# bleyerj/dolfinx_materials

Hardware: AMD Instinct MI355X
Metric: M quadrature-point updates/s (stress+tangent, fp64) (higher is better)
Workload: dtype f64; 1 GPU; cfg2: J2 von-Mises plasticity, linear isotropic hardening, small strain, 1e+07 Gauss points per GPU, stress + 6x6 consistent tangent, load/unload history increments 2-4; points_per_gpu=10000000, law=j2_linear, layout=AoS (N,6)/(N,36) boundary arrays in HBM, SoA resident state, placement=every array where its first allocation put it, settle_launches_before_warmup=540

## Files before the change

dolfinx_materials_amd/_lib.py:

```python
from __future__ import annotations

import ctypes as C
import os
import subprocess

_HERE = os.path.dirname(os.path.abspath(__file__))
LIB_PATH = os.environ.get("DXM_LIB_PATH") or os.path.join(_HERE, "libdxmat.so")
CSRC_DIR = os.path.join(_HERE, "csrc")

DXM_MAX_STATE_FIELDS = 4
LAW_ELASTIC_ISO, LAW_J2_LINEAR, LAW_J2_VOCE, LAW_FEFP_J2_VOCE, LAW_FEFP_J2_LINEAR = 0, 1, 2, 3, 4
LAW_RAMBERG_OSGOOD = 5
LAW_OGDEN = 7
LAW_HOSFORD_LINEAR = 10
LAW_ORTHOTROPIC_ELASTIC = 12
S0, S1 = 0, 1


class DxmError(RuntimeError):
    """Hard error reported by libdxmat (negative return code)."""


class LawInfo(C.Structure):
    _fields_ = [
# ... 41 lines not shown
    "dxm_destroy": (C.c_int, [_h]),
    "dxm_npoints": (C.c_int64, [_h]),
    "dxm_law": (C.c_int, [_h]),
    "dxm_set_params": (C.c_int, [_h, _dp, C.c_int]),
    "dxm_set_param_field": (C.c_int, [_h, C.c_int, C.c_void_p]),
    "dxm_set_param_field_device": (C.c_int, [_h, C.c_int, C.c_void_p, C.c_void_p]),
    "dxm_param_field_mask": (C.c_int, [_h]),
    "dxm_set_frame": (C.c_int, [_h, C.c_void_p]),
    "dxm_set_frame_field": (C.c_int, [_h, C.c_void_p]),
    "dxm_set_frame_field_device": (C.c_int, [_h, C.c_void_p, C.c_void_p]),
    "dxm_frame_kind": (C.c_int, [_h]),
    "dxm_algorithmic_bytes": (C.c_int, [_h]),
    "dxm_set_newton": (C.c_int, [_h, C.c_int, C.c_double]),
    "dxm_set_tangent_layout": (C.c_int, [_h, C.c_int]),
    "dxm_tangent_size": (C.c_int, [_h]),
    "dxm_set_state": (C.c_int, [_h, C.c_int, C.c_int, C.c_void_p]),
    "dxm_get_state": (C.c_int, [_h, C.c_int, C.c_int, C.c_void_p]),
    "dxm_advance": (C.c_int, [_h]),
    "dxm_revert": (C.c_int, [_h]),
    "dxm_io_held": (C.c_int, [_h, C.c_int]),
    "dxm_get_io": (C.c_int, [_h, C.c_int, C.c_int, C.c_void_p]),
    "dxm_integrate_rows": (C.c_int, [_h, C.c_void_p, C.c_double, C.c_void_p, C.c_void_p, C.c_void_p, C.POINTER(Stats)]),
    "dxm_integrate": (
        C.c_int,
        [_h, C.c_void_p, C.c_double, C.c_void_p, C.c_void_p, C.c_void_p, C.POINTER(Stats)],
    ),
    "dxm_integrate_device": (
        C.c_int,
        [_h, C.c_void_p, C.c_double, C.c_void_p, C.c_void_p, C.c_void_p],
    ),
    "dxm_get_stats": (C.c_int, [_h, C.POINTER(Stats)]),
    "dxm_isv_device": (C.c_int, [_h, C.c_int, C.c_void_p, C.c_void_p]),
    "dxm_state_ptr": (C.c_void_p, [_h, C.c_int, C.c_int, C.c_int]),
    "dxm_integrate_displacement_device": (C.c_int, [_h, _h, C.c_void_p, C.c_double, C.c_void_p, C.c_void_p, C.c_void_p]),
    "dxm_expand_tangent_device": (C.c_int, [C.c_void_p, C.c_int64, C.c_void_p, C.c_int, C.c_void_p]),
    "dxm_expand_tangent_pack4_device": (C.c_int, [C.c_void_p, C.c_void_p, C.c_int64, C.c_void_p, C.c_int, C.c_void_p]),
    "dxm_kernel_name": (C.c_char_p, [_h]),
    "dxm_launch_generation": (C.c_uint64, [_h]),
    "dxm_notify_replay": (C.c_int, [_h]),
    "dxm_set_option": (C.c_int, [_h, C.c_char_p, C.c_double]),
    "dxm_isv_host": (C.c_int, [_h, C.c_int, C.c_void_p]),
    "dxm_bind_isv_output": (C.c_int, [_h, C.c_int, C.c_void_p]),
    "dxm_host_copy": (C.c_int, [C.c_void_p, C.c_void_p, C.c_uint64, C.c_int]),
    "dxm_host_scatter_rows": (C.c_int, [C.c_void_p, C.c_void_p, C.c_void_p, C.c_int64, C.c_int, C.c_int]),
    "dxm_host_gather_rows": (C.c_int, [C.c_void_p, C.c_void_p, C.c_void_p, C.c_int64, C.c_int, C.c_int]),
    "dxm_host_index_range": (C.c_int, [C.c_void_p, C.c_int64, C.c_int, C.POINTER(C.c_int64), C.POINTER(C.c_int64)]),
    "dxm_host_register": (C.c_int, [C.c_void_p, C.c_uint64]),
    "dxm_host_unregister": (C.c_int, [C.c_void_p]),
    "dxm_host_alloc": (C.c_void_p, [C.c_uint64]),
    "dxm_host_free": (C.c_int, [C.c_void_p]),
    "dxm_mesh_create_hex8": (_h, [C.c_void_p, C.c_int64, C.c_void_p, C.c_int64, C.c_void_p, C.c_int, C.c_int]),
    "dxm_mesh_create_tet4": (_h, [C.c_void_p, C.c_int64, C.c_void_p, C.c_int64, C.c_int, C.c_int]),
    "dxm_mesh_create_simplex": (
        _h,
        [C.c_int, C.c_void_p, C.c_int64, C.c_void_p, C.c_int64, C.c_void_p, C.c_int, C.c_int64, C.c_void_p, C.c_int, C.c_int],
    ),
    "dxm_mesh_destroy": (C.c_int, [_h]),
    "dxm_mesh_npoints": (C.c_int64, [_h]),
    "dxm_mesh_displacement_size": (C.c_int64, [_h]),
    "dxm_mesh_gradient_device": (C.c_int, [_h, C.c_void_p, C.c_int, C.c_void_p, C.c_void_p]),
    "dxm_integrate_displacement": (
        C.c_int,
        [_h, _h, C.c_void_p, C.c_double, C.c_void_p, C.c_void_p, C.c_void_p, C.POINTER(Stats)],
    ),
    "dxm_integrate_displacement_rows": (
        C.c_int,
# ... 197 lines not shown
```

dolfinx_materials_amd/csrc/dxmat.hip:

```cpp
#include <hip/hip_runtime.h>

#include <algorithm>
#include <atomic>
#include <chrono>
#include <cmath>
#include <condition_variable>
#include <deque>
#include <map>
#include <mutex>
#include <thread>
#include <cstdarg>
#include <cstdio>
#include <cstdlib>
#include <cstring>
#include <string>
#include <vector>

#include "../../include/dxmat.h"
#include "dxm_common.hpp"
#include "fefp.hpp"
#include "gradient.hpp"
#include "small_strain.hpp"
#include "ramberg_osgood.hpp"
#include "param_fields.hpp"
#include "hyperelastic.hpp"
#include "hosford.hpp"
#include "orthotropic.hpp"
#include "host_side.hpp"

using namespace dxm;
static_assert(TL_FULL == DXM_TANGENT_FULL && TL_SYM == DXM_TANGENT_SYM && TL_COEF == DXM_TANGENT_COEF && TL_PACK4 == DXM_TANGENT_PACK4, "kernel and ABI layout ids");

static thread_local std::string g_last_error;

static int fail(int code, const char* fmt, ...) {
  char buf[512];
  va_list ap;
  va_start(ap, fmt);
  vsnprintf(buf, sizeof(buf), fmt, ap);
  va_end(ap);
  g_last_error = buf;
  return code;
}

#define HIP_TRY(expr)                                                                      \
  do {                                                                                     \
    hipError_t _e = (expr);                                                                \
    if (_e != hipSuccess) {                                                                \
      (void)hipGetLastError();                                                             \
      return fail(-2, "%s failed: %s (%s:%d)", #expr, hipGetErrorString(_e), __FILE__, __LINE__); \
    }                                                                                      \
  } while (0)

struct DeviceGuard {
  int prev = -1;
  bool ok = true;
// ... 444 lines not shown
  double* h_coef = nullptr;
  int h_coef_per_point = 0;
  double* h_flux = nullptr;
  double* h_isv = nullptr;
  double elastic_lm[2] = {0.0, 0.0};
  hipEvent_t chunk_done[DXM_MAX_CHUNKS] = {};
  hipEvent_t kernel_done[DXM_MAX_CHUNKS] = {};
  int num_cu = 256;
  int blocks_per_cu = 5;
  int tangent_layout = 0;
  double* d_grad = nullptr;
  double* d_flux = nullptr;
  double* d_grad0 = nullptr;
  double* d_flux0 = nullptr;
  int io1_valid = 0;
  int io0_valid = 0;
  int opt_keep_initial_io = 0;
  double* d_isv = nullptr;
  double* isv_out[DXM_MAX_STATE_FIELDS] = {};
  double* d_isv_fields = nullptr;
  double* d_ct = nullptr;
  double* d_field = nullptr;
  double* h_grad_ring = nullptr;
  int64_t ring_slot_doubles = 0;
  hipEvent_t ring_done[DXM_RING] = {};
  int opt_stage_ahead = 3;
  double unregister_ms = 0.0;
  int pf_mask = 0;
  double* pf_law[2] = {nullptr, nullptr};
  double* pf_stream[PF_COUNT] = {};
  int frame_kind = 0;
  Frame9 frame_uniform{};
  double* frame_streams = nullptr;
};

static int sync_last(dxm_material* m);
static int pf_refresh_elastic(dxm_material* m, hipStream_t st);

static void free_state(dxm_material* m) {
  if (!m->state_base) return;
  (void)hipFree(m->state_base);
  m->state_base = nullptr;
}

static int build_params(dxm_material* m, const double* p, int np) {
  const LawDesc& d = kLaws[m->law];
  const int expect = n_params_of(d);
  if (np != expect) return fail(-1, "law %d expects %d parameters, got %d", m->law, expect, np);
  LawParams q{};
  q.maxit = m->maxit;
  q.rtol = m->rtol;
  if (int rc = d.build(p, q)) return rc;
  m->prm = q;
  m->raw_params.assign(p, p + np);
  return 0;
}

static int tangent_size(const dxm_material* m) {
  const LawDesc& d = kLaws[m->law];
  if (m->tangent_layout == DXM_TANGENT_SYM) return d.n_flux * (d.n_flux + 1) / 2;
  if (m->tangent_layout == DXM_TANGENT_COEF) return 9;
  if (m->tangent_layout == DXM_TANGENT_PACK4) return 4;
  return d.n_flux * d.n_grad;
}

__global__ void fill_slot_kernel(double* dst, int64_t count, double value) {
  const int64_t i = (int64_t)blockIdx.x * blockDim.x + threadIdx.x;
  if (i < count) dst[i] = value;
}

struct PackMap { int n; int slot[16]; };

// ... 100 lines not shown
  if (hipStreamCreateWithFlags(&m->own_stream, hipStreamNonBlocking) != hipSuccess ||
      hipEventCreateWithFlags(&m->last_event, hipEventDisableTiming) != hipSuccess) {
    fail(-2, "hipStreamCreate / hipEventCreate failed"); return bail();
  }
  if (d.n_slots > 0) {
    const size_t bytes = (size_t)d.n_slots * m->ld * sizeof(double);
    {
      if (hipMalloc(&m->state_base, 2 * bytes + m->s1_skew) != hipSuccess) {
        fail(-3, "hipMalloc of %zu state bytes failed", 2 * bytes + m->s1_skew); return bail();
      }
      m->state[0] = m->state_base;
      m->state[1] = reinterpret_cast<double*>(reinterpret_cast<char*>(m->state_base) + bytes + m->s1_skew);
    }
  }
  {
    hipFuncAttributes fa;
    if (d.residency_kernel && hipFuncGetAttributes(&fa, d.residency_kernel()) == hipSuccess && fa.numRegs > 0) {
      const int alloc = ((fa.numRegs + 7) / 8) * 8;
      int waves_simd = 512 / alloc;
      if (waves_simd > 8) waves_simd = 8;
      int by_vgpr = waves_simd * 4 / WAVES_PER_BLOCK;
      int by_lds = fa.sharedSizeBytes > 0 ? (int)(160 * 1024 / fa.sharedSizeBytes) : 8;
      int occ = by_vgpr < by_lds ? by_vgpr : by_lds;
      if (occ < 1) occ = 1;
      m->blocks_per_cu = occ;
    }
    if (d.blocks_per_cu) m->blocks_per_cu = d.blocks_per_cu;
  }
  m->stats_capacity = dxm_host::stats_capacity(m->num_cu, npoints);
  if (hipMalloc(&m->d_stats, sizeof(BlockStats) * m->stats_capacity) != hipSuccess) {
    fail(-3, "hipMalloc of stats failed"); return bail();
  }
  if (init_state(m) != 0) return bail();
  g_last_error.clear();
  return m;
}

int dxm_destroy(dxm_material* m) {
  if (!m) return 0;
  DeviceGuard guard(m->device);
  (void)sync_last(m);
  delete m->pool;
  if (m->h_coef) (void)hipHostFree(m->h_coef);
  if (m->h_flux) (void)hipHostFree(m->h_flux);
  if (m->h_isv) (void)hipHostFree(m->h_isv);
  for (hipEvent_t e : m->chunk_done) if (e) (void)hipEventDestroy(e);
  for (hipEvent_t e : m->kernel_done) if (e) (void)hipEventDestroy(e);
  if (m->last_event) (void)hipEventDestroy(m->last_event);
  free_state(m);
  if (m->d_stats) (void)hipFree(m->d_stats);
  if (m->h_stats) (void)hipHostFree(m->h_stats);
  if (m->d_grad) (void)hipFree(m->d_grad);
  if (m->d_flux) (void)hipFree(m->d_flux);
  if (m->d_grad0) (void)hipFree(m->d_grad0);
  if (m->d_flux0) (void)hipFree(m->d_flux0);
  if (m->d_isv) (void)hipFree(m->d_isv);
  if (m->d_isv_fields) (void)hipFree(m->d_isv_fields);
  if (m->d_ct) (void)hipFree(m->d_ct);
  if (m->d_field) (void)hipFree(m->d_field);
  if (m->h_grad_ring) (void)hipHostFree(m->h_grad_ring);
  for (double* q : m->pf_law) if (q) (void)hipFree(q);
  for (double* q : m->pf_stream) if (q) (void)hipFree(q);
  if (m->frame_streams) (void)hipFree(m->frame_streams);
  for (hipEvent_t e : m->ring_done) if (e) (void)hipEventDestroy(e);
  if (m->own_stream) (void)hipStreamDestroy(m->own_stream);
  if (m->pipe_stream) (void)hipStreamDestroy(m->pipe_stream);
// ... 36 lines not shown
  if (maxit < 1 || !(rtol > 0.0)) return fail(-1, "invalid Newton controls maxit=%d rtol=%g", maxit, rtol);
  m->maxit = maxit;
  m->rtol = rtol;
  if (int rc = build_params(m, m->raw_params.data(), (int)m->raw_params.size())) return rc;
  ++m->epoch;
  return 0;
}

static int check_field(const dxm_material* m, int which, int field) {
  if (!m) return fail(-1, "null handle");
  if (which != DXM_S0 && which != DXM_S1) return fail(-1, "state selector must be DXM_S0 or DXM_S1");
  const LawDesc& d = kLaws[m->law];
  if (field < 0 || field >= d.n_fields) return fail(-1, "law %d has no state field %d", m->law, field);
  return 0;
}

static int sync_last(dxm_material* m) {
  if (!m->launched) return 0;
  if (m->last_event_recorded) {
    HIP_TRY(hipEventSynchronize(m->last_event));
  } else {
    HIP_TRY(hipDeviceSynchronize());
  }
  return 0;
}

static double* state_of(const dxm_material* m, int which) {
  return m->state[(which == DXM_S1 && !m->s1_alias) ? 1 : 0];
}

static int materialize_s1(dxm_material* m) {
  if (!m->s1_alias) return 0;
  const LawDesc& d = kLaws[m->law];
  if (d.n_slots > 0)
    HIP_TRY(hipMemcpy(m->state[1], m->state[0], (size_t)d.n_slots * m->ld * sizeof(double),
                      hipMemcpyDeviceToDevice));
  m->s1_alias = false;
  return 0;
}


constexpr size_t BOUNCE_BYTES = 16u << 20;
static dxm_host::LockedTable g_locked;
static std::atomic<int> g_query_foreign{1};
static void note_locked(const void* p, size_t bytes) { g_locked.note(p, bytes); }
static void forget_locked(const void* p) { g_locked.forget(p); }
static bool in_locked_table(const void* host, size_t bytes) { return g_locked.contains(host, bytes); }
static bool page_locked_byte(const void* host) {
  hipPointerAttribute_t attr{};
  const bool locked = host && hipPointerGetAttributes(&attr, host) == hipSuccess && attr.type == hipMemoryTypeHost;
  (void)hipGetLastError();
  return locked;
}
static bool page_locked(const void* host, size_t bytes) {
  if (!host) return false;
  if (in_locked_table(host, bytes)) return true;
  if (!g_query_foreign.load()) return false;
  if (!page_locked_byte(host)) return false;
  return bytes <= 1 || page_locked_byte(static_cast<const char*>(host) + bytes - 1);
}
struct Staging {
  char* buf = nullptr;
  hipEvent_t done[2] = {nullptr, nullptr};
};
static std::mutex g_staging_mu[64];
static Staging g_staging[64];
// ... 53 lines not shown
  if (int rc = current_device_index(&devi)) return rc;
  std::lock_guard<std::mutex> lk(g_staging_mu[devi]);
  Staging* s = nullptr;
  if (int rc = staging_for_current_device(&s)) return rc;
  const size_t nchunks = (bytes + BOUNCE_BYTES - 1) / BOUNCE_BYTES;
  for (size_t c = 0; c < nchunks; ++c) {
    if (c >= 2) HIP_TRY(hipEventSynchronize(s->done[c & 1]));
    memcpy(s->buf + (c & 1) * BOUNCE_BYTES, static_cast<const char*>(host) + c * BOUNCE_BYTES, chunk_size(c, nchunks, bytes));
    HIP_TRY(hipMemcpyAsync(static_cast<char*>(dev) + c * BOUNCE_BYTES, s->buf + (c & 1) * BOUNCE_BYTES, chunk_size(c, nchunks, bytes),
                           hipMemcpyHostToDevice, st));
    HIP_TRY(hipEventRecord(s->done[c & 1], st));
  }
  HIP_TRY(hipStreamSynchronize(st));
  return 0;
}

int dxm_set_state(dxm_material* m, int which, int field, const double* host_aos) {
  if (int rc = check_field(m, which, field)) return rc;
  if (!host_aos) return fail(-1, "null host pointer");
  DEVICE_GUARD(m);
  if (int rc = sync_last(m)) return rc;
  const LawDesc& d = kLaws[m->law];
  const int dim = d.isv_dim[field];
  const int64_t n = m->n;
  if (n == 0) return 0;
  if (int rc = materialize_s1(m)) return rc;
  if (!m->d_field) HIP_TRY(hipMalloc(&m->d_field, sizeof(double) * n * 6));
  PackMap map{};
  map.n = dim;
  for (int c = 0; c < dim; ++c) map.slot[c] = d.isv_slot[field] + c;
  hipStream_t st = m->own_stream;
  if (int rc = upload_from_host(m->d_field, host_aos, sizeof(double) * n * dim, st)) return rc;
  const int blocks = (int)((n * dim + 255) / 256);
  hipLaunchKernelGGL(unpack_isv_kernel, dim3(blocks), dim3(256), 0, st, state_of(m, which), m->ld, n,
                     m->d_field, map);
  HIP_TRY(hipGetLastError());
  HIP_TRY(hipStreamSynchronize(st));
  return 0;
}

int dxm_get_state(dxm_material* m, int which, int field, double* host_aos) {
  if (int rc = check_field(m, which, field)) return rc;
  if (!host_aos) return fail(-1, "null host pointer");
  DEVICE_GUARD(m);
  if (int rc = sync_last(m)) return rc;
  const LawDesc& d = kLaws[m->law];
  const int dim = d.isv_dim[field];
  const int64_t n = m->n;
  if (n == 0) return 0;
  if (!m->d_field) HIP_TRY(hipMalloc(&m->d_field, sizeof(double) * n * 6));
  PackMap map{};
  map.n = dim;
  for (int c = 0; c < dim; ++c) map.slot[c] = d.isv_slot[field] + c;
  hipStream_t st = m->own_stream;
  const int blocks = (int)((n * dim + 255) / 256);
  hipLaunchKernelGGL(pack_isv_kernel, dim3(blocks), dim3(256), 0, st, state_of(m, which), m->ld, n,
                     m->d_field, map);
  HIP_TRY(hipGetLastError());
  return download_to_host(host_aos, m->d_field, sizeof(double) * n * dim, st);
}

int dxm_advance(dxm_material* m) {
  if (!m) return fail(-1, "null handle");
  if (!m->s1_alias) {
    double* t = m->state[0];
    m->state[0] = m->state[1];
// ... 27 lines not shown
  if (!host_aos) return fail(-1, "null host pointer");
  DEVICE_GUARD(m);
  if (int rc = sync_last(m)) return rc;
  const LawDesc& d = kLaws[m->law];
  const bool first = which == DXM_S0 || m->s1_alias;
  const double* src = kind ? (first ? m->d_flux0 : m->d_flux) : (first ? m->d_grad0 : m->d_grad);
  return download_to_host(host_aos, src, sizeof(double) * m->n * (kind ? d.n_flux : d.n_grad), m->own_stream);
}

int dxm_revert(dxm_material* m) {
  if (!m) return fail(-1, "null handle");
  m->s1_alias = true;
  m->io1_valid = 0;
  return 0;
}

}

template <int LAW>
static void launch_small_strain(const LaunchArgs& a) {
  dxm_material* m = a.m;
  const int grid = a.grid, tl = a.tl;
  const hipStream_t st = a.st;
  const int64_t cnt = a.cnt;
  const double* grad = a.grad;
  double *flux = a.flux, *ct = a.ct;
  const double* s0 = m->state[0] + a.off;
  double* s1 = m->state[1] + a.off;
  BlockStats* bs = m->d_stats + a.stats_off;
  const MeshSource none{};
  const MeshSource& src = a.fused ? *a.fused : none;
  const int g = a.fused ? a.fused->kind : 0;
  constexpr int dyn_lds = LAW == LAW_ELASTIC ? 0 : 2304;
#ifndef DXM_CUSTOM_HARDENING
  if constexpr (LAW != LAW_ELASTIC) {
    if (m->pf_mask) {
      ParamStreams pf{};
      for (int k = 0; k < PF_COUNT; ++k) pf.p[k] = m->pf_stream[k] ? m->pf_stream[k] + a.off : nullptr;
      param_fields_launch(LAW, tl, g, grid, dyn_lds, st, m->prm, pf, cnt, grad, s0, s1, m->ld, flux, ct, bs, src);
      return;
    }
  }
#endif
#define DXM_LAUNCH_SS(TL, G)                                                                              \
  hipLaunchKernelGGL((small_strain_kernel<LAW, TL, G>), dim3(grid), dim3(BLOCK), dyn_lds, st, m->prm, cnt, grad, s0, s1, \
                     m->ld, flux, ct, bs, src)
#define DXM_LAUNCH_SS_G(TL) do { if (g == 0) DXM_LAUNCH_SS(TL, 0); else if (g == 1) DXM_LAUNCH_SS(TL, 1); \
                                 else if (g == 2) DXM_LAUNCH_SS(TL, 2); else DXM_LAUNCH_SS(TL, 3); } while (0)
  if (tl == TL_SYM) DXM_LAUNCH_SS_G(TL_SYM);
  else if (tl == TL_FULL) DXM_LAUNCH_SS_G(TL_FULL);
  else if constexpr (ss_has_coef<LAW>) { if (tl == TL_PACK4) DXM_LAUNCH_SS_G(TL_PACK4); else DXM_LAUNCH_SS_G(TL_COEF); }
#undef DXM_LAUNCH_SS_G
#undef DXM_LAUNCH_SS
}

static void launch_fefp(const LaunchArgs& a, bool voce) {
  dxm_material* m = a.m;
  const int grid = a.grid;
  const hipStream_t st = a.st;
  const int64_t cnt = a.cnt;
  const double* grad = a.grad;
  double *flux = a.flux, *ct = a.ct;
  const double* s0 = m->state[0] + a.off;
  double* s1 = m->state[1] + a.off;
  BlockStats* bs = m->d_stats + a.stats_off;
  const MeshSource none{};
// ... 737 lines not shown

int dxm_integrate_displacement_rows(dxm_material* m, dxm_mesh* mesh, const double* u_host, double dt, double* flux_rows,
                                    double* ct_rows, const int64_t* rows, dxm_stats* stats) {
  (void)dt;
  if (!m) return fail(-1, "null argument");
  if (m->n > 0 && (!flux_rows || !ct_rows || !rows)) return fail(-1, "dxm_integrate_displacement_rows needs the flux array, the tangent array and the row index");
  return integrate_displacement_host(m, mesh, u_host, flux_rows, nullptr, ct_rows, stats, rows);
}

int dxm_integrate_displacement_device(dxm_material* m, dxm_mesh* mesh, const double* u_dev, double dt,
                                      double* flux_dev, double* ct_dev, void* hip_stream) {
  (void)dt;
  if (!m || !mesh) return fail(-1, "null argument");
  if (mesh->device != m->device) return fail(-1, "mesh and material live on different devices");
  if (dxm_mesh_npoints(mesh) != m->n) return fail(-1, "mesh has %lld Gauss points, material %lld",
                                                   (long long)dxm_mesh_npoints(mesh), (long long)m->n);
  if (m->n > 0 && (!u_dev || !flux_dev || !ct_dev)) return fail(-1, "null device pointer");
  DEVICE_GUARD(m);
  hipStream_t st = (hipStream_t)hip_stream;
  const LawDesc& d = kLaws[m->law];
  if (m->opt_fused_gradient && fusable(mesh)) {
    const MeshSource src = mesh_source(mesh, u_dev);
    return launch(m, flux_dev , flux_dev, ct_dev, st, &src);
  }
  if (!m->d_grad) HIP_TRY(hipMalloc(&m->d_grad, sizeof(double) * m->n * d.n_grad));
  if (int rc = dxm_mesh_gradient_device(mesh, u_dev, gradient_kind(d), m->d_grad, hip_stream)) return rc;
  return launch(m, m->d_grad, flux_dev, ct_dev, st);
}

const double* dxm_state_ptr(const dxm_material* m, int which, int field, int comp) {
  if (check_field(m, which, field)) return nullptr;
  const LawDesc& d = kLaws[m->law];
  if (comp < 0 || comp >= d.isv_dim[field]) { fail(-1, "component out of range"); return nullptr; }
  return state_of(m, which) + (size_t)(d.isv_slot[field] + comp) * m->ld;
}

const char* dxm_kernel_name(const dxm_material* m) {
  if (!m) return "";
  if (m->frame_kind) return kLaws[m->law].frame_kernel[m->frame_kind - 1];
  return m->pf_mask ? kLaws[m->law].field_kernel : kLaws[m->law].kernel;
}

int dxm_expand_tangent_device(const double* coef_dev, int64_t npoints, double* ct_dev, int device, void* hip_stream) {
  if (npoints < 0) return fail(-1, "negative point count");
  if (npoints == 0) return 0;
  if (!coef_dev || !ct_dev) return fail(-1, "null device pointer");
  if (((uintptr_t)coef_dev | (uintptr_t)ct_dev) & 15) return fail(-1, "coefficient / tangent device arrays must be 16-byte aligned");
  DeviceGuard guard(device);
  if (!guard.ok) return fail(-2, "hipSetDevice(%d) failed", device);
  const int64_t tiles = (npoints + WAVE - 1) / WAVE;
  int64_t blocks = (tiles + WAVES_PER_BLOCK - 1) / WAVES_PER_BLOCK;
  if (blocks > 256 * 32) blocks = 256 * 32;
  hipLaunchKernelGGL(expand_tangent_kernel, dim3((unsigned)blocks), dim3(BLOCK), 0, (hipStream_t)hip_stream, npoints, coef_dev, ct_dev);
  HIP_TRY(hipGetLastError());
  return 0;
}

int dxm_expand_tangent_pack4_device(const double* flux_dev, const double* pack_dev, int64_t npoints, double* ct_dev, int device,
                                    void* hip_stream) {
  if (npoints < 0) return fail(-1, "negative point count");
  if (npoints == 0) return 0;
  if (!flux_dev || !pack_dev || !ct_dev) return fail(-1, "null device pointer");
  if (((uintptr_t)flux_dev | (uintptr_t)pack_dev | (uintptr_t)ct_dev) & 15) return fail(-1, "stress / pack / tangent device arrays must be 16-byte aligned");
  DeviceGuard guard(device);
  if (!guard.ok) return fail(-2, "hipSetDevice(%d) failed", device);
  const int64_t tiles = (npoints + WAVE - 1) / WAVE;
  int64_t blocks = (tiles + WAVES_PER_BLOCK - 1) / WAVES_PER_BLOCK;
// ... 204 lines not shown

int dxm_set_frame_field_device(dxm_material* m, const double* dev_aos, void* hip_stream) {
  if (int rc = frame_check(m)) return rc;
  if (!dev_aos) return dxm_set_frame_field(m, nullptr);
  DEVICE_GUARD(m);
  hipStream_t st = (hipStream_t)hip_stream;
  if (m->launched && m->last_event_recorded) HIP_TRY(hipStreamWaitEvent(st, m->last_event, 0));
  else if (int rc = sync_last(m)) return rc;
#ifndef DXM_CUSTOM_HARDENING
  if (int rc = frame_reserve(m)) return rc;
  orthotropic_frames_to_streams(m->n, dev_aos, m->frame_streams, m->ld, st);
  HIP_TRY(hipGetLastError());
#endif
  m->frame_kind = 2;
  ++m->epoch;
  return 0;
}

int dxm_frame_kind(const dxm_material* m) { return m ? m->frame_kind : -1; }

int dxm_algorithmic_bytes(const dxm_material* m) {
  if (!m) return -1;
  int bytes = kLaws[m->law].alg_bytes;
  for (const double* q : m->pf_stream) if (q) bytes += 8;
  if (m->frame_kind == 2) bytes += 9 * 8;
  return bytes;
}

int dxm_notify_replay(dxm_material* m) {
  if (!m) return fail(-1, "null handle");
  m->launched = true;
  m->last_event_recorded = false;
  m->s1_alias = false;
  return 0;
}

uint64_t dxm_launch_generation(const dxm_material* m) { return m ? (m->epoch << 1) | (uint64_t)m->parity : 0; }

int dxm_set_option(dxm_material* m, const char* name, double value) {
  if (!m || !name) return fail(-1, "null argument");
  const std::string k(name);
  const bool on = value != 0.0;
  if (k == "pipeline") m->opt_pipeline = on;
  else if (k == "split_streams") m->opt_split_streams = on;
  else if (k == "packed_transfer") {
    if (!(value == 0.0 || value == 1.0 || value == 2.0)) return fail(-1, "packed_transfer must be 0, 1 or 2");
    m->opt_packed_transfer = (int)value;
  }
  else if (k == "fused_gradient") m->opt_fused_gradient = on;
  else if (k == "verbose") m->opt_verbose = on;
  else if (k == "stage_ahead") {
    if (!(value >= 1 && value <= DXM_RING - 2)) return fail(-1, "stage_ahead must be in [1, %d]", DXM_RING - 2);
    m->opt_stage_ahead = (int)value;
  }
  else if (k == "register_input") {
    if (!(value == 0.0 || value == 1.0 || value == 2.0)) return fail(-1, "register_input must be 0, 1 or 2");
    m->up.set_option((int)value);
  }
  else if (k == "keep_initial_io") m->opt_keep_initial_io = on;
  else if (k == "pageable_dma") m->opt_pageable_dma = value != 0.0;
  else if (k == "query_foreign_pointers") g_query_foreign.store(on ? 1 : 0);
  else if (k == "packed_min_points") {
    if (!(value >= 0 && value <= 1e12)) return fail(-1, "packed_min_points must be >= 0");
    m->opt_packed_min_points = (int64_t)value;
  }
  else if (k == "host_threads") {
    if (!(value >= 1 && value <= 256)) return fail(-1, "host_threads must be in [1, 256]");
    m->opt_host_threads = (int)value;
  } else if (k == "max_chunks") {
    if (!(value >= 1 && value <= DXM_MAX_CHUNKS)) return fail(-1, "max_chunks must be in [1, %d]", DXM_MAX_CHUNKS);
    m->opt_max_chunks = (int)value;
  } else if (k == "blocks_per_cu") {
    if (!(value >= 1 && value <= 256)) return fail(-1, "blocks_per_cu must be in [1, 256]");
    m->blocks_per_cu = (int)value;
  } else {
    return fail(-1, "unknown option '%s'", name);
  }
  ++m->epoch;
  return 0;
}

int dxm_isv_host(dxm_material* m, int which, double* isv_aos) {
  if (!m) return fail(-1, "null handle");
  if (which != DXM_S0 && which != DXM_S1) return fail(-1, "state selector must be DXM_S0 or DXM_S1");
  const LawDesc& d = kLaws[m->law];
  const int total = isv_total(d);
  if (total == 0 || m->n == 0) return 0;
  if (!isv_aos) return fail(-1, "null host pointer");
  DEVICE_GUARD(m);
  if (int rc = sync_last(m)) return rc;
  if (!m->d_isv) HIP_TRY(hipMalloc(&m->d_isv, sizeof(double) * m->n * total));
  if (int rc = pack_isv_range(m, which, 0, m->n, m->d_isv, m->own_stream)) return rc;
  return download_to_host(isv_aos, m->d_isv, sizeof(double) * m->n * total, m->own_stream);
}

int dxm_host_copy(void* dst, const void* src, uint64_t bytes, int threads) {
  if (bytes == 0) return 0;
  if (!dst || !src) return fail(-1, "null host pointer");
  dxm_host::host_copy(dst, src, bytes, threads);
  return 0;
}

static int move_rows(bool scatter, double* dst, const double* src, const int64_t* rows, int64_t n, int width, int threads) {
  if (n <= 0 || width <= 0) return 0;
  if (!dst || !src || !rows) return fail(-1, "null host pointer");
  dxm_host::move_rows(scatter, dst, src, rows, n, width, threads);
  return 0;
// ... 38 lines not shown
```

dolfinx_materials_amd/csrc/host_side.hpp:

```cpp
#pragma once

#include <algorithm>
#include <atomic>
#include <cmath>
#include <condition_variable>
#include <cstdint>
#include <cstring>
#include <deque>
#include <map>
#include <mutex>
#include <thread>
#include <vector>

#include "../../include/dxmat.h"

namespace dxm_host {

typedef double double2_h __attribute__((ext_vector_type(2)));

constexpr double THIRD = 1.0 / 3.0;
constexpr int MAX_CHUNKS = 64;
constexpr int RING = 16;
constexpr int FEFP_RECORD = 54;

// ... 229 lines not shown
};

struct ChunkPlan {
  int nchunks;
  int64_t csize;
  int64_t offset(int c) const { return (int64_t)c * csize; }
  int64_t count(int c, int64_t n) const {
    const int64_t o = offset(c);
    return o >= n ? 0 : ((n - o) < csize ? (n - o) : csize);
  }
  int issued(int64_t n) const { return csize > 0 ? (int)std::min<int64_t>(nchunks, (n + csize - 1) / csize) : 0; }
};

inline ChunkPlan plan_chunks(int64_t n, bool packed, bool staged_upload, int max_chunks, bool pipeline) {
  int nchunks = (int)std::min<int64_t>(n / (packed ? (n >= 2097152 ? 65536 : 32768) : 131072), MAX_CHUNKS * 1024);
  if (nchunks < 1) nchunks = 1;
  if (!packed && nchunks > (staged_upload ? 32 : 8)) nchunks = staged_upload ? 32 : 8;
  if (nchunks > max_chunks) nchunks = max_chunks;
  if (nchunks > MAX_CHUNKS) nchunks = MAX_CHUNKS;
  if (!pipeline) nchunks = 1;
  const int64_t csize = ((n + nchunks - 1) / nchunks + 255) / 256 * 256;
  return ChunkPlan{nchunks, csize};
}

inline int ring_slot(int chunk) { return chunk % RING; }

inline int stats_capacity(int num_cu, int64_t npoints) {
  return (int)std::min<int64_t>(INT32_MAX, std::max<int64_t>((int64_t)num_cu * 256, (npoints + 255) / 256 + MAX_CHUNKS));
}
inline int launch_grid(int64_t cnt, int num_cu, int blocks_per_cu) {
  const int64_t tiles = (cnt + 255) / 256;
  const int64_t cap = (int64_t)num_cu * blocks_per_cu;
  return (int)std::max<int64_t>(1, std::min<int64_t>(tiles, cap));
}

struct TransferRequest {
  int law;
  int n_grad, n_flux, n_isv_fields, isv_dim[DXM_MAX_STATE_FIELDS];
  int layout, tangent_size;
  int64_t n;
  bool flux, isv_aos, ct;
  bool rows;
  bool staged_grad;
  bool fused;
  unsigned bound_fields;
  bool flux_locked, isv_locked, ct_locked;
  int packed_transfer;
  int64_t packed_min_points;
  bool split_streams, pipeline;
  int max_chunks;
};

enum class Route { none, dma, staged, rows };
enum class CtRoute { none, fill, dma, staged, rebuild, rows_move, rows_rebuild, rows_fill };

struct TransferPlan {
  TransferRequest req;
  bool packed;
  int tl;
  int nt;
  int np;
  int land;
  int nfull;
  int job;
  CtRoute ct;
  Route flux, isv, fields;
// ... 227 lines not shown
```

dolfinx_materials_amd/csrc/small_strain.hpp:

```cpp
#pragma once
#include "dxm_common.hpp"
#include "gradient.hpp"
#include "param_fields.hpp"

namespace dxm {

enum { LAW_ELASTIC = 0, LAW_J2_LINEAR = 1, LAW_J2_VOCE = 2, LAW_RAMBERG_OSGOOD = 3 };

template <int LAW> constexpr bool ss_has_state = LAW == LAW_J2_LINEAR || LAW == LAW_J2_VOCE;
template <int LAW> constexpr bool ss_has_coef = LAW != LAW_ELASTIC;

constexpr int RO_I3MU = 0, RO_BETA = 1, RO_ISIG0 = 2, RO_N = 3, RO_INVN = 4, RO_ESIG = 5;
constexpr double RO_EPS = 1e-12;

constexpr int SS_NSLOTS = 7;

constexpr int SS_STAGE = 64 * 6;
constexpr int SS_COEF = 64 * 9;
constexpr int SS_LDS_PER_WAVE = SS_STAGE + SS_COEF;
static_assert(8 * HEX_FUSED_REC <= SS_COEF, "the 8 cell records of a fused tile live in the coefficient region");

template <int LAW>
__device__ __forceinline__ double hardening_R(const LawParams& prm, double p) {
  if constexpr (LAW == LAW_J2_LINEAR) {
// ... 77 lines not shown
  const double d[6] = {et[0] - third, et[1] - third, et[2] - third, et[3], et[4], et[5]};
  const double g = se * (2.0 / 3.0) / fmax(eq, RO_EPS);
  const double ktr = prm.kappa * tr;
  s[0] = ktr + g * d[0];
  s[1] = ktr + g * d[1];
  s[2] = ktr + g * d[2];
  s[3] = g * d[3];
  s[4] = g * d[4];
  s[5] = g * d[5];
}

__device__ __forceinline__ double2_t tangent_pair(const double* cf, int i, int j) {
  const double k1 = cf[0], k2 = cf[1], k3 = cf[2];
  const double ni = cf[3 + i], nj0 = cf[3 + j], nj1 = cf[4 + j];
  const double t0 = ((i < 3 && j < 3) ? k1 : 0.0) + ((i == j) ? k2 : 0.0);
  const double t1 = ((i < 3 && j + 1 < 3) ? k1 : 0.0) + ((i == j + 1) ? k2 : 0.0);
  double2_t v;
  v.x = t0 + k3 * (ni * nj0);
  v.y = t1 + k3 * (ni * nj1);
  return v;
}

enum { TL_FULL = 0, TL_SYM = 1, TL_COEF = 2, TL_PACK4 = 3 };
constexpr double SS_THIRD = 1.0 / 3.0;

template <int LAW, int TL, int GRAD = 0>
__global__ void __launch_bounds__(BLOCK, 4)
small_strain_kernel(const LawParams prm, const int64_t n, const double* __restrict__ eps,
                    const double* __restrict__ s0, double* __restrict__ s1, const int64_t ld,
                    double* __restrict__ sig, double* __restrict__ ct,
                    BlockStats* __restrict__ stats, const MeshSource src) {
  constexpr bool FIELDS = false;
  constexpr ParamStreams pf = {};
#include "small_strain_body.hpp"
}

template <int LAW, int TL, int GRAD = 0>
__global__ void __launch_bounds__(BLOCK, 4)
small_strain_field_kernel(const LawParams prm, const ParamStreams pf, const int64_t n, const double* __restrict__ eps,
                          const double* __restrict__ s0, double* __restrict__ s1, const int64_t ld,
                          double* __restrict__ sig, double* __restrict__ ct,
                          BlockStats* __restrict__ stats, const MeshSource src) {
  static_assert(LAW == LAW_J2_LINEAR || LAW == LAW_J2_VOCE, "parameter fields: the J2 laws");
  constexpr bool FIELDS = true;
#include "small_strain_body.hpp"
}

#ifndef DXM_UPDATE_KERNELS_ONLY
__global__ void __launch_bounds__(BLOCK, 4)
expand_tangent_kernel(const int64_t n, const double* __restrict__ cin, double* __restrict__ ct) {
  __shared__ __attribute__((aligned(16))) double lds_all[WAVES_PER_BLOCK * SS_COEF];
  const int lane = threadIdx.x & (WAVE - 1);
  const int wid = threadIdx.x >> 6;
  double* coef = lds_all + wid * SS_COEF;
  const int64_t ntiles = (n + WAVE - 1) / WAVE;
  for (int64_t tile = (int64_t)blockIdx.x * WAVES_PER_BLOCK + wid; tile < ntiles; tile += (int64_t)gridDim.x * WAVES_PER_BLOCK) {
    const int64_t base = tile * WAVE;
    const int npts = (n - base) < WAVE ? (int)(n - base) : WAVE;
    if (npts == WAVE) {
      const double2_t* g = reinterpret_cast<const double2_t*>(cin + base * 9);
      double2_t v[5];
#pragma unroll
      for (int k = 0; k < 5; ++k) v[k] = (k * WAVE + lane < 288) ? g[k * WAVE + lane] : double2_t{0.0, 0.0};
#pragma unroll
      for (int k = 0; k < 5; ++k)
        if (k * WAVE + lane < 288) reinterpret_cast<double2_t*>(coef)[k * WAVE + lane] = v[k];
    } else {
#pragma unroll
      for (int k = 0; k < 9; ++k) {
        const int idx = k * WAVE + lane;
        coef[idx] = idx < npts * 9 ? cin[base * 9 + idx] : 0.0;
      }
    }
    wave_lds_sync();
#include "small_strain_expand_store.hpp"
    wave_lds_sync();
  }
// ... 46 lines not shown
```

dolfinx_materials_amd/csrc/small_strain_body.hpp:

```cpp
  __shared__ __attribute__((aligned(16))) double lds_all[WAVES_PER_BLOCK * SS_LDS_PER_WAVE];
  __shared__ unsigned long long red[4 * WAVES_PER_BLOCK];

  int lane = threadIdx.x & (WAVE - 1);
  const int wid = threadIdx.x >> 6;
  double* stage = lds_all + wid * SS_LDS_PER_WAVE;
  double* coef = stage + SS_STAGE;
  double2_t* stage2 = reinterpret_cast<double2_t*>(stage);

  const int64_t ntiles = (n + WAVE - 1) / WAVE;
  const int64_t tile_stride = (int64_t)gridDim.x * WAVES_PER_BLOCK;

  unsigned long long c_plastic = 0, c_notconv = 0, c_nan = 0, c_maxit = 0;

  const double lambda_u = prm.lambda, mu_u = prm.mu;

  for (int64_t tile = (int64_t)blockIdx.x * WAVES_PER_BLOCK + wid; tile < ntiles;
       tile += tile_stride) {
    const int64_t base = tile * WAVE;
    const int npts = (n - base) < WAVE ? (int)(n - base) : WAVE;
    if constexpr (FIELDS || LAW == LAW_J2_VOCE || LAW == LAW_RAMBERG_OSGOOD) {
      asm volatile("" : "+v"(lane));
      lane &= WAVE - 1;
    }
    const bool valid = lane < npts;
    const int64_t gi = base + lane;

    double e[6];
    double p_n = 0.0, ep[6] = {0, 0, 0, 0, 0, 0};
    if constexpr (GRAD == 0) {
#include "tile_rows6_load.hpp"
      if constexpr (ss_has_state<LAW>) {
        if (valid) {
          p_n = stream_load<3>(s0 + gi);
#pragma unroll
          for (int c = 0; c < 6; ++c) ep[c] = stream_load<3>(s0 + (int64_t)(1 + c) * ld + gi);
        }
      }
      wave_lds_sync();
#include "tile_rows6_take.hpp"
      wave_lds_sync();
    } else {
      double Hd[9];
      if constexpr (GRAD == 1) {
        {
          const int64_t cell = ((src.point0 + base) >> 3) + (lane >> 3);
          double2_t r0 = {0.0, 0.0}, r1 = {0.0, 0.0}, r2 = {0.0, 0.0};
          if (cell < src.ncells) {
            const int64_t nd = src.conn[cell * 8 + (lane & 7)];
            r0 = double2_t{src.coords[3 * nd], src.coords[3 * nd + 1]};
            r1 = double2_t{src.coords[3 * nd + 2], src.u[3 * nd]};
            r2 = double2_t{src.u[3 * nd + 1], src.u[3 * nd + 2]};
          }
          double2_t* d = reinterpret_cast<double2_t*>(coef + (lane >> 3) * HEX_FUSED_REC + (lane & 7) * 6);
          d[0] = r0; d[1] = r1; d[2] = r2;
        }
        wave_lds_sync();
        {
          const double2_t* rec = reinterpret_cast<const double2_t*>(coef + (lane >> 3) * HEX_FUSED_REC);
          auto node = [&](int m, double* X, double* U) {
            const double2_t a = rec[m * 3], b = rec[m * 3 + 1], c = rec[m * 3 + 2];
            X[0] = a.x; X[1] = a.y; X[2] = b.x;
            U[0] = b.y; U[1] = c.x; U[2] = c.y;
          };
          const int q = lane & 7;
          if (valid) {
            hex8_disp_grad(src.xi[q][0], src.xi[q][1], src.xi[q][2], node, Hd);
          } else {
#pragma unroll
            for (int k = 0; k < 9; ++k) Hd[k] = 0.0;
          }
// ... 70 lines not shown
            if (fabs(r) <= tolp) break;
            if (it >= prm.maxit) { if (valid) ++c_notconv; break; }
            const double dr = -3.0 * mu - hardening_dR<LAW>(lp, p_n + dp);
            dp -= r / dr;
            ++iters;
          }
        }
        const double iseq = 1.0 / seq;
        double nn[6];
#pragma unroll
        for (int c = 0; c < 6; ++c) nn[c] = 1.5 * se[c] * iseq;
        const double beta = dp * iseq;
        {
          const double rho = 1.0 - 3.0 * mu * beta;
          wn = rho > 0.0 ? 1.5 * iseq / rho : 0.0;
          if constexpr (LAW != LAW_J2_LINEAR) { if (valid && !(rho > 0.0)) ++c_notconv; }
          else if ((FIELDS && pf.p[PF_H1]) ? lp.h1 < 0.0 : prm.h1 < 0.0) { if (valid && !(rho > 0.0)) ++c_notconv; }
        }
        const double gamma = 1.0 / (hardening_dR<LAW>(lp, p_n + dp) + 3.0 * mu);
        c1 = lambda + 2.0 * mu * mu * beta;
        c2 = 2.0 * mu - 6.0 * mu * mu * beta;
        c3 = 4.0 * mu * mu * (beta - gamma);
        p_new = p_n + dp;
#pragma unroll
        for (int c = 0; c < 6; ++c) {
          ep[c] += dp * nn[c];
          e[c] -= dp * nn[c];
        }
        if (valid) {
          ++c_plastic;
          c_maxit = iters > c_maxit ? iters : c_maxit;
        }
      }
    }
    const double ltr = lambda * (e[0] + e[1] + e[2]);
    double s[6];
    if constexpr (LAW == LAW_RAMBERG_OSGOOD) {
      ramberg_osgood_update(prm, mu, e, stage2 + lane * 3, s, c1, c2, c3, wn, valid, c_plastic, c_notconv, c_maxit);
    } else {
    s[0] = ltr + 2.0 * mu * e[0];
    s[1] = ltr + 2.0 * mu * e[1];
    s[2] = ltr + 2.0 * mu * e[2];
    s[3] = 2.0 * mu * e[3];
    s[4] = 2.0 * mu * e[4];
    s[5] = 2.0 * mu * e[5];
    }
    {
      const double chk = s[0] + s[1] + s[2] + s[3] + s[4] + s[5] + p_new + ((c1 + c2) + (c3 + wn));
      if (valid && !(fabs(chk) <= 1.79769313486231570e308)) ++c_nan;
    }

    if constexpr (ss_has_state<LAW>) {
      if (valid) {
        stream_store<1>(s1 + gi, p_new);
#pragma unroll
        for (int c = 0; c < 6; ++c) stream_store<1>(s1 + (int64_t)(1 + c) * ld + gi, ep[c]);
      }
    }

    stage2[lane * 3 + 0] = double2_t{s[0], s[1]};
    stage2[lane * 3 + 1] = double2_t{s[2], s[3]};
    stage2[lane * 3 + 2] = double2_t{s[4], s[5]};
    if constexpr (ss_has_coef<LAW> && TL == TL_PACK4) {
      double2_t* c4 = reinterpret_cast<double2_t*>(coef) + lane * 2;
      c4[0] = double2_t{c1, c2};
      c4[1] = double2_t{c3, wn};
    } else if constexpr (ss_has_coef<LAW>) {
#include "small_strain_stage_coef.hpp"
    }
    wave_lds_sync();

#include "tile_rows6_store.hpp"
    if constexpr (TL == TL_PACK4) {
      static_assert(ss_has_coef<LAW>, "the elastic tangent is a constant: nothing to write");
      if (npts == WAVE) {
        double2_t* gct = reinterpret_cast<double2_t*>(ct + base * 4);
        const double2_t* c4 = reinterpret_cast<const double2_t*>(coef);
        stream_store<0>(gct + lane, c4[lane]);
        stream_store<0>(gct + WAVE + lane, c4[WAVE + lane]);
      } else {
        double2_t* gct = reinterpret_cast<double2_t*>(ct + base * 4);
        const double2_t* c4 = reinterpret_cast<const double2_t*>(coef);
        if (lane < npts * 2) stream_store<0>(gct + lane, c4[lane]);
        if (WAVE + lane < npts * 2) stream_store<0>(gct + WAVE + lane, c4[WAVE + lane]);
      }
    } else if constexpr (TL == TL_COEF) {
      static_assert(ss_has_coef<LAW>, "the elastic tangent is a constant: nothing to write");
      if (npts == WAVE) {
        double2_t* gct = reinterpret_cast<double2_t*>(ct + base * 9);
// ... 90 lines not shown
```

include/dxmat.h:

```cpp
#ifndef DXMAT_H
#define DXMAT_H

#include <stdint.h>

#ifdef __cplusplus
extern "C" {
#endif

#define DXM_ABI_VERSION 6

enum {
  DXM_LAW_ELASTIC_ISO = 0,
  DXM_LAW_J2_LINEAR = 1,
  DXM_LAW_J2_VOCE = 2,
  DXM_LAW_FEFP_J2_VOCE = 3,
  DXM_LAW_FEFP_J2_LINEAR = 4,
  DXM_LAW_RAMBERG_OSGOOD = 5,
  DXM_LAW_OGDEN = 7,
  DXM_LAW_HOSFORD_LINEAR = 10,
  DXM_LAW_ORTHOTROPIC_ELASTIC = 12,
  DXM_LAW_COUNT = 13
};

enum { DXM_S0 = 0, DXM_S1 = 1 };
// ... 36 lines not shown
int dxm_set_param_field(dxm_material* m, int param_index, const double* host_values);
int dxm_set_param_field_device(dxm_material* m, int param_index, const double* dev_values, void* hip_stream);
int dxm_param_field_mask(const dxm_material* m);
int dxm_set_frame(dxm_material* m, const double* r9);
int dxm_set_frame_field(dxm_material* m, const double* host_aos);
int dxm_set_frame_field_device(dxm_material* m, const double* dev_aos, void* hip_stream);
int dxm_frame_kind(const dxm_material* m);
int dxm_algorithmic_bytes(const dxm_material* m);
enum { DXM_UPLOAD_NONE = 0, DXM_UPLOAD_PAGE_LOCKED = 1 ,
       DXM_UPLOAD_REGISTERED = 2 ,
       DXM_UPLOAD_STAGED = 3 ,
       DXM_UPLOAD_RUNTIME = 4  };
enum { DXM_TANGENT_FULL = 0, DXM_TANGENT_SYM = 1, DXM_TANGENT_COEF = 2, DXM_TANGENT_PACK4 = 3 };
int dxm_set_tangent_layout(dxm_material* m, int layout);
int dxm_tangent_size(const dxm_material* m);
int dxm_set_newton(dxm_material* m, int maxit, double rtol);

int dxm_set_state(dxm_material* m, int which, int field, const double* host_aos);
int dxm_get_state(dxm_material* m, int which, int field, double* host_aos);
int dxm_advance(dxm_material* m);
int dxm_revert(dxm_material* m);
int dxm_io_held(const dxm_material* m, int which);
int dxm_get_io(dxm_material* m, int which, int kind, double* host_aos);

int dxm_integrate(dxm_material* m, const double* grad_aos, double dt, double* flux_aos,
                  double* isv_aos, double* ct_aos, dxm_stats* stats);
int dxm_integrate_rows(dxm_material* m, const double* grad_aos, double dt, double* flux_rows, double* ct_rows,
                       const int64_t* rows, dxm_stats* stats);
int dxm_integrate_device(dxm_material* m, const double* grad_dev, double dt, double* flux_dev,
                         double* ct_dev, void* hip_stream);
int dxm_get_stats(dxm_material* m, dxm_stats* stats);
int dxm_isv_device(dxm_material* m, int which, double* isv_aos_dev, void* hip_stream);
const double* dxm_state_ptr(const dxm_material* m, int which, int field, int comp);
int dxm_expand_tangent_device(const double* coef_dev, int64_t npoints, double* ct_dev, int device, void* hip_stream);
int dxm_expand_tangent_pack4_device(const double* flux_dev, const double* pack_dev, int64_t npoints, double* ct_dev, int device,
                                    void* hip_stream);
const char* dxm_kernel_name(const dxm_material* m);
uint64_t dxm_launch_generation(const dxm_material* m);
int dxm_notify_replay(dxm_material* m);
int dxm_set_option(dxm_material* m, const char* name, double value);
int dxm_isv_host(dxm_material* m, int which, double* isv_aos);
int dxm_bind_isv_output(dxm_material* m, int field, double* host_aos);

void* dxm_host_alloc(uint64_t bytes);
int dxm_host_free(void* p);
int dxm_host_copy(void* dst, const void* src, uint64_t bytes, int threads);
int dxm_host_scatter_rows(double* dst, const double* src, const int64_t* rows, int64_t n, int width, int threads);
int dxm_host_gather_rows(double* dst, const double* src, const int64_t* rows, int64_t n, int width, int threads);
int dxm_host_index_range(const int64_t* rows, int64_t n, int threads, int64_t* lo, int64_t* hi);
int dxm_host_register(void* p, uint64_t bytes);
int dxm_host_unregister(void* p);

typedef struct dxm_mesh dxm_mesh;
dxm_mesh* dxm_mesh_create_hex8(const double* coords, int64_t n_nodes, const int32_t* conn,
                               int64_t n_cells, const double* qpoints, int nqp, int device);
dxm_mesh* dxm_mesh_create_tet4(const double* coords, int64_t n_nodes, const int32_t* conn,
                               int64_t n_cells, int nqp, int device);
dxm_mesh* dxm_mesh_create_simplex(int tdim, const double* coords, int64_t n_vertices, const int32_t* geom_conn,
                                  int64_t n_cells, const int32_t* dofmap, int nd, int64_t n_dofs,
                                  const double* dphi, int nqp, int device);
int dxm_mesh_destroy(dxm_mesh* mesh);
int64_t dxm_mesh_npoints(const dxm_mesh* mesh);
int64_t dxm_mesh_displacement_size(const dxm_mesh* mesh);
int dxm_mesh_gradient_device(dxm_mesh* mesh, const double* u_dev, int kind, double* grad_dev,
                             void* hip_stream);
int dxm_integrate_displacement(dxm_material* m, dxm_mesh* mesh, const double* u_host, double dt,
// ... 13 lines not shown
```

Baseline: 10690 Mpoints/s.

## Skip state writeback for elastic wave tiles using per-tile clean stamps

Adds a per-64-point-tile stamp array and a specialised J2 kernel that skips writing the new plastic state (p, eps_p) when every point in a wave tile stayed elastic and the tile was already marked clean for the current stamp. Stamps are bumped on advance, state upload and option changes, and cleared on wraparound. This cuts HBM store traffic for the seven state fields. In exchange it adds a stamp read, a ballot and host-side launch selection logic, and correctness depends on s1 still holding valid data from earlier steps.

```diff
diff --git a/dolfinx_materials_amd/_lib.py b/dolfinx_materials_amd/_lib.py
--- a/dolfinx_materials_amd/_lib.py
+++ b/dolfinx_materials_amd/_lib.py
@@ -97,6 +97,7 @@
     "dxm_get_stats": (C.c_int, [_h, C.POINTER(Stats)]),
     "dxm_isv_device": (C.c_int, [_h, C.c_int, C.c_void_p, C.c_void_p]),
     "dxm_state_ptr": (C.c_void_p, [_h, C.c_int, C.c_int, C.c_int]),
+    "dxm_clean_tiles": (C.c_int, [_h, C.POINTER(C.c_int64), C.POINTER(C.c_int64)]),
     "dxm_integrate_displacement_device": (C.c_int, [_h, _h, C.c_void_p, C.c_double, C.c_void_p, C.c_void_p, C.c_void_p]),
     "dxm_expand_tangent_device": (C.c_int, [C.c_void_p, C.c_int64, C.c_void_p, C.c_int, C.c_void_p]),
     "dxm_expand_tangent_pack4_device": (C.c_int, [C.c_void_p, C.c_void_p, C.c_int64, C.c_void_p, C.c_int, C.c_void_p]),
diff --git a/dolfinx_materials_amd/csrc/dxmat.hip b/dolfinx_materials_amd/csrc/dxmat.hip
--- a/dolfinx_materials_amd/csrc/dxmat.hip
+++ b/dolfinx_materials_amd/csrc/dxmat.hip
@@ -22,6 +22,7 @@
 #include "gradient.hpp"
 #include "small_strain.hpp"
 #include "ramberg_osgood.hpp"
+#include "small_strain_clean.hpp"
 #include "param_fields.hpp"
 #include "hyperelastic.hpp"
 #include "hosford.hpp"
@@ -532,12 +533,26 @@
   int frame_kind = 0;
   Frame9 frame_uniform{};
   double* frame_streams = nullptr;
+  uint32_t* stamps = nullptr;
+  uint32_t clean_stamp = 1;
+  bool stamps_stale = false;
+  bool opt_elide_clean_state = true;
+  mutable bool state_exposed = false;
 };
 
 static int sync_last(dxm_material* m);
 static int pf_refresh_elastic(dxm_material* m, hipStream_t st);
 
+static void bump_clean_stamp(dxm_material* m) {
+  if (!m->stamps) return;
+  bool wrapped = false;
+  m->clean_stamp = dxm_host::next_clean_stamp(m->clean_stamp, &wrapped);
+  if (wrapped) m->stamps_stale = true;
+}
+static int64_t stamp_words(const dxm_material* m) { return (m->ld + 63) / 64; }
+
 static void free_state(dxm_material* m) {
+  if (m->stamps) { (void)hipFree(m->stamps); m->stamps = nullptr; }
   if (!m->state_base) return;
   (void)hipFree(m->state_base);
   m->state_base = nullptr;
@@ -704,6 +719,14 @@
     fail(-3, "hipMalloc of stats failed"); return bail();
   }
   if (init_state(m) != 0) return bail();
+#ifndef DXM_CUSTOM_HARDENING
+  if (law == DXM_LAW_J2_LINEAR || law == DXM_LAW_J2_VOCE) {
+    const size_t bytes = sizeof(uint32_t) * (size_t)stamp_words(m);
+    if (hipMalloc(&m->stamps, bytes) != hipSuccess || hipMemset(m->stamps, 0, bytes) != hipSuccess) {
+      fail(-3, "hipMalloc / hipMemset of %zu stamp bytes failed", bytes); return bail();
+    }
+  }
+#endif
   g_last_error.clear();
   return m;
 }
@@ -806,6 +829,7 @@
 static int materialize_s1(dxm_material* m) {
   if (!m->s1_alias) return 0;
   const LawDesc& d = kLaws[m->law];
+  bump_clean_stamp(m);
   if (d.n_slots > 0)
     HIP_TRY(hipMemcpy(m->state[1], m->state[0], (size_t)d.n_slots * m->ld * sizeof(double),
                       hipMemcpyDeviceToDevice));
@@ -925,6 +949,7 @@
   hipStream_t st = m->own_stream;
   if (int rc = upload_from_host(m->d_field, host_aos, sizeof(double) * n * dim, st)) return rc;
   const int blocks = (int)((n * dim + 255) / 256);
+  bump_clean_stamp(m);
   hipLaunchKernelGGL(unpack_isv_kernel, dim3(blocks), dim3(256), 0, st, state_of(m, which), m->ld, n,
                      m->d_field, map);
   HIP_TRY(hipGetLastError());
@@ -1018,6 +1043,39 @@
   const MeshSource& src = a.fused ? *a.fused : none;
   const int g = a.fused ? a.fused->kind : 0;
   constexpr int dyn_lds = LAW == LAW_ELASTIC ? 0 : 2304;
+  if constexpr (ss_has_state<LAW>) {
+    if (m->stamps) {
+      hipStreamCaptureStatus cap = hipStreamCaptureStatusNone;
+      if (hipStreamIsCapturing(st, &cap) != hipSuccess) { (void)hipGetLastError(); cap = hipStreamCaptureStatusActive; }
+      const bool capturing = cap != hipStreamCaptureStatusNone;
+      if (m->stamps_stale && !capturing && m->opt_elide_clean_state && !m->state_exposed) {
+        if (sync_last(m) == 0 && hipMemsetAsync(m->stamps, 0, sizeof(uint32_t) * (size_t)stamp_words(m), st) == hipSuccess) {
+          m->stamps_stale = false;
+          m->clean_stamp = 1;
+        } else {
+          (void)hipGetLastError();
+        }
+      }
+      dxm_host::StateLaunchFlags f{};
+      f.has_stamps = true;
+      f.option = m->opt_elide_clean_state;
+      f.fields = m->pf_mask != 0;
+      f.frame = m->frame_kind != 0;
+      f.fused = a.fused != nullptr;
+      f.whole_tiles = dxm_host::covers_whole_tiles(a.off, cnt, m->n);
+      f.capturing = capturing;
+      f.exposed = m->state_exposed;
+      f.stamps_stale = m->stamps_stale;
+      const dxm_host::StateLaunch how = dxm_host::choose_state_launch(f);
+#ifndef DXM_CUSTOM_HARDENING
+      if (how == dxm_host::StateLaunch::clean &&
+          small_strain_clean_launch(LAW, tl, grid, dyn_lds, st, m->prm, cnt, grad, s0, s1, m->ld, flux, ct, bs, m->stamps + a.off / WAVE,
+                                    m->clean_stamp))
+        return;
+#endif
+      bump_clean_stamp(m);
+    }
+  }
 #ifndef DXM_CUSTOM_HARDENING
   if constexpr (LAW != LAW_ELASTIC) {
     if (m->pf_mask) {
@@ -1821,7 +1879,25 @@
   if (check_field(m, which, field)) return nullptr;
   const LawDesc& d = kLaws[m->law];
   if (comp < 0 || comp >= d.isv_dim[field]) { fail(-1, "component out of range"); return nullptr; }
+  m->state_exposed = true;
   return state_of(m, which) + (size_t)(d.isv_slot[field] + comp) * m->ld;
+}
+
+int dxm_clean_tiles(dxm_material* m, int64_t* clean, int64_t* tiles) {
+  if (!m || !clean || !tiles) return fail(-1, "null argument");
+  *clean = *tiles = 0;
+  if (!m->stamps || m->n == 0) return 0;
+  DEVICE_GUARD(m);
+  if (int rc = sync_last(m)) return rc;
+  const int64_t nt = (m->n + WAVE - 1) / WAVE;
+  *tiles = nt;
+  if (!m->opt_elide_clean_state || m->state_exposed || m->stamps_stale) return 0;
+  std::vector<uint32_t> host((size_t)nt);
+  if (int rc = download_to_host(host.data(), m->stamps, sizeof(uint32_t) * (size_t)nt, m->own_stream)) return rc;
+  int64_t c = 0;
+  for (uint32_t v : host) c += v == m->clean_stamp;
+  *clean = c;
+  return 0;
 }
 
 const char* dxm_kernel_name(const dxm_material* m) {
@@ -2092,6 +2168,7 @@
   m->launched = true;
   m->last_event_recorded = false;
   m->s1_alias = false;
+  bump_clean_stamp(m);
   return 0;
 }
 
@@ -2133,6 +2210,9 @@
   } else if (k == "blocks_per_cu") {
     if (!(value >= 1 && value <= 256)) return fail(-1, "blocks_per_cu must be in [1, 256]");
     m->blocks_per_cu = (int)value;
+  } else if (k == "elide_clean_state") {
+    m->opt_elide_clean_state = on;
+    bump_clean_stamp(m);
   } else {
     return fail(-1, "unknown option '%s'", name);
   }
diff --git a/dolfinx_materials_amd/csrc/host_side.hpp b/dolfinx_materials_amd/csrc/host_side.hpp
--- a/dolfinx_materials_amd/csrc/host_side.hpp
+++ b/dolfinx_materials_amd/csrc/host_side.hpp
@@ -285,6 +285,30 @@
   const int64_t tiles = (cnt + 255) / 256;
   const int64_t cap = (int64_t)num_cu * blocks_per_cu;
   return (int)std::max<int64_t>(1, std::min<int64_t>(tiles, cap));
+}
+
+enum class StateLaunch { clean, plain, plain_bump };
+struct StateLaunchFlags {
+  bool has_stamps;
+  bool option;
+  bool fields;
+  bool frame;
+  bool fused;
+  bool whole_tiles;
+  bool capturing;
+  bool exposed;
+  bool stamps_stale;
+};
+inline StateLaunch choose_state_launch(const StateLaunchFlags& f) {
+  if (!f.has_stamps) return StateLaunch::plain;
+  if (f.option && !f.fields && !f.frame && !f.fused && f.whole_tiles && !f.capturing && !f.exposed && !f.stamps_stale) return StateLaunch::clean;
+  return StateLaunch::plain_bump;
+}
+inline bool covers_whole_tiles(int64_t off, int64_t cnt, int64_t npoints) { return off % 64 == 0 && (cnt % 64 == 0 || off + cnt == npoints); }
+inline uint32_t next_clean_stamp(uint32_t s, bool* wrapped) {
+  const uint32_t t = s + 1u;
+  *wrapped = t == 0u;
+  return t == 0u ? 1u : t;
 }
 
 struct TransferRequest {
diff --git a/dolfinx_materials_amd/csrc/small_strain.hpp b/dolfinx_materials_amd/csrc/small_strain.hpp
--- a/dolfinx_materials_amd/csrc/small_strain.hpp
+++ b/dolfinx_materials_amd/csrc/small_strain.hpp
@@ -133,6 +133,9 @@
                     BlockStats* __restrict__ stats, const MeshSource src) {
   constexpr bool FIELDS = false;
   constexpr ParamStreams pf = {};
+  constexpr bool CLEAN = false;
+  constexpr uint32_t* stamps = nullptr;
+  constexpr uint32_t stamp = 0;
 #include "small_strain_body.hpp"
 }
 
@@ -144,6 +147,9 @@
                           BlockStats* __restrict__ stats, const MeshSource src) {
   static_assert(LAW == LAW_J2_LINEAR || LAW == LAW_J2_VOCE, "parameter fields: the J2 laws");
   constexpr bool FIELDS = true;
+  constexpr bool CLEAN = false;
+  constexpr uint32_t* stamps = nullptr;
+  constexpr uint32_t stamp = 0;
 #include "small_strain_body.hpp"
 }
 
diff --git a/dolfinx_materials_amd/csrc/small_strain_body.hpp b/dolfinx_materials_amd/csrc/small_strain_body.hpp
--- a/dolfinx_materials_amd/csrc/small_strain_body.hpp
+++ b/dolfinx_materials_amd/csrc/small_strain_body.hpp
@@ -24,6 +24,8 @@
     }
     const bool valid = lane < npts;
     const int64_t gi = base + lane;
+    [[maybe_unused]] uint32_t tile_stamp = 0;
+    [[maybe_unused]] bool any_plastic = true;
 
     double e[6];
     double p_n = 0.0, ep[6] = {0, 0, 0, 0, 0, 0};
@@ -36,6 +38,7 @@
           for (int c = 0; c < 6; ++c) ep[c] = stream_load<3>(s0 + (int64_t)(1 + c) * ld + gi);
         }
       }
+      if constexpr (CLEAN) tile_stamp = __builtin_amdgcn_readfirstlane(stamps[tile]);
       wave_lds_sync();
 #include "tile_rows6_take.hpp"
       wave_lds_sync();
@@ -172,6 +175,7 @@
           c_maxit = iters > c_maxit ? iters : c_maxit;
         }
       }
+      if constexpr (CLEAN) any_plastic = __ballot(valid && f > 0.0) != 0;
     }
     const double ltr = lambda * (e[0] + e[1] + e[2]);
     double s[6];
@@ -191,10 +195,16 @@
     }
 
     if constexpr (ss_has_state<LAW>) {
-      if (valid) {
+      if (CLEAN ? (valid && (any_plastic || tile_stamp != stamp)) : valid) {
         stream_store<1>(s1 + gi, p_new);
 #pragma unroll
         for (int c = 0; c < 6; ++c) stream_store<1>(s1 + (int64_t)(1 + c) * ld + gi, ep[c]);
+      }
+      if constexpr (CLEAN) {
+        if (lane == 0) {
+          if (any_plastic) { if (tile_stamp == stamp) stamps[tile] = 0u; }
+          else if (tile_stamp != stamp) stamps[tile] = stamp;
+        }
       }
     }
 
diff --git a/dolfinx_materials_amd/csrc/small_strain_clean.hip b/dolfinx_materials_amd/csrc/small_strain_clean.hip
--- /dev/null
+++ b/dolfinx_materials_amd/csrc/small_strain_clean.hip
@@ -0,0 +1,40 @@
+#include "small_strain_clean.hpp"
+
+#define DXM_UPDATE_KERNELS_ONLY
+#include "small_strain.hpp"
+
+namespace dxm {
+
+template <int LAW, int TL, int GRAD = 0>
+__global__ void __launch_bounds__(BLOCK, 4)
+small_strain_clean_kernel(const LawParams prm, const int64_t n, const double* __restrict__ eps,
+                          const double* __restrict__ s0, double* __restrict__ s1, const int64_t ld,
+                          double* __restrict__ sig, double* __restrict__ ct,
+                          BlockStats* __restrict__ stats, uint32_t* __restrict__ stamps, const uint32_t stamp) {
+  static_assert(ss_has_state<LAW> && GRAD == 0, "the J2 laws, strain from the (N, 6) array");
+  constexpr bool FIELDS = false;
+  constexpr ParamStreams pf = {};
+  constexpr bool CLEAN = true;
+  MeshSource src{};
+#include "small_strain_body.hpp"
+}
+
+const void* small_strain_clean_kernel_ptr() { return (const void*)small_strain_clean_kernel<LAW_J2_LINEAR, TL_FULL>; }
+
+bool small_strain_clean_launch(int law, int tl, int grid, int dyn_lds, hipStream_t st, const LawParams& prm, int64_t cnt,
+                               const double* grad, const double* s0, double* s1, int64_t ld, double* flux, double* ct,
+                               BlockStats* bs, uint32_t* stamps, uint32_t stamp) {
+#define DXM_LAUNCH_CLEAN(LAW, TL)                                                                                      \
+  hipLaunchKernelGGL((small_strain_clean_kernel<LAW, TL>), dim3(grid), dim3(BLOCK), dyn_lds, st, prm, cnt, grad, s0, s1, ld, \
+                     flux, ct, bs, stamps, stamp)
+#define DXM_LAUNCH_CLEAN_TL(LAW) do { if (tl == TL_SYM) DXM_LAUNCH_CLEAN(LAW, TL_SYM); else if (tl == TL_FULL) DXM_LAUNCH_CLEAN(LAW, TL_FULL); \
+                                      else if (tl == TL_PACK4) DXM_LAUNCH_CLEAN(LAW, TL_PACK4); else DXM_LAUNCH_CLEAN(LAW, TL_COEF); } while (0)
+  if (law == LAW_J2_LINEAR) DXM_LAUNCH_CLEAN_TL(LAW_J2_LINEAR);
+  else if (law == LAW_J2_VOCE) DXM_LAUNCH_CLEAN_TL(LAW_J2_VOCE);
+  else return false;
+#undef DXM_LAUNCH_CLEAN_TL
+#undef DXM_LAUNCH_CLEAN
+  return true;
+}
+
+}
diff --git a/dolfinx_materials_amd/csrc/small_strain_clean.hpp b/dolfinx_materials_amd/csrc/small_strain_clean.hpp
--- /dev/null
+++ b/dolfinx_materials_amd/csrc/small_strain_clean.hpp
@@ -0,0 +1,14 @@
+#pragma once
+#include <hip/hip_runtime.h>
+
+#include "dxm_common.hpp"
+
+namespace dxm {
+
+__attribute__((visibility("hidden"))) const void* small_strain_clean_kernel_ptr();
+
+__attribute__((visibility("hidden"))) bool small_strain_clean_launch(int law, int tl, int grid, int dyn_lds, hipStream_t st, const LawParams& prm,
+                                                                     int64_t cnt, const double* grad, const double* s0, double* s1, int64_t ld,
+                                                                     double* flux, double* ct, BlockStats* bs, uint32_t* stamps, uint32_t stamp);
+
+}
diff --git a/include/dxmat.h b/include/dxmat.h
--- a/include/dxmat.h
+++ b/include/dxmat.h
@@ -92,6 +92,7 @@
 int dxm_get_stats(dxm_material* m, dxm_stats* stats);
 int dxm_isv_device(dxm_material* m, int which, double* isv_aos_dev, void* hip_stream);
 const double* dxm_state_ptr(const dxm_material* m, int which, int field, int comp);
+int dxm_clean_tiles(dxm_material* m, int64_t* clean, int64_t* tiles);
 int dxm_expand_tangent_device(const double* coef_dev, int64_t npoints, double* ct_dev, int device, void* hip_stream);
 int dxm_expand_tangent_pack4_device(const double* flux_dev, const double* pack_dev, int64_t npoints, double* ct_dev, int device,
                                     void* hip_stream);
```

Result: faster. 11110 Mpoints/s, median of 6 (+3.9%).
